# meyerls/FruitNeRF

Measured on AMD Instinct MI355X. Metric: train rays/sec, fruit_nerf on synthetic apple 800x800, higher is better.
Workload: dtype f32 fwd (MLP GEMMs: 3-piece bf16 split, 6 products, ~2^-24) / 2-piece bwd (dX, dW: 3 products, ~2^-17; its forward recompute 3-piece); everything else f32

## Files before the change

fruitnerf_amd/csrc/hash_scatter.hip:

```cpp
#include <stdlib.h>
#include <string.h>

#include "hash_scatter.hpp"
#include "sequencer.hpp"

namespace fnr {

constexpr int SC_MAX_ROWS = 8192;
constexpr int SC_MAX_BINS = 256;
constexpr int SC_CHUNK = 512;
constexpr int SC_EMIT_THREADS = 512;
constexpr int SC_PER_THREAD = SC_CHUNK / SC_EMIT_THREADS;
constexpr int SC_BINS_PER_THREAD = 1;
static_assert(SC_MAX_BINS <= SC_EMIT_THREADS, "one bin per thread");
constexpr int SC_CNT_STRIDE = 32;

__device__ unsigned long long g_scatter_overflow_records;
__device__ unsigned long long g_scatter_records[2][64][16];



struct ScatterPlan {
  int log2_rows;
  int bins_per_level;
// ... 52 lines not shown
  bool any_run;
};
template <int CTRL>
__device__ __forceinline__ float dpp_shr0_f32(float v) {
  return __builtin_bit_cast(float, __builtin_amdgcn_update_dpp(0, __builtin_bit_cast(int, v), CTRL, 0xf, 0xf, true));
}
__device__ __forceinline__ RunMasks run_structure(uint32_t key_a, uint32_t key_b, int lane) {
  const int j = lane & 15;
  const uint32_t pa = dpp_u32<0x111>(~key_a, key_a), pb = dpp_u32<0x111>(key_b, key_b);
  const bool head = (pa != key_a) || (pb != key_b);
  const unsigned long long heads = __ballot(head);
  const uint32_t row = (uint32_t)(heads >> (lane & 48)) & 0xffffu;
  const uint32_t below = row & ((2u << j) - 1u);
  const int dist = j - (31 - __clz((int)below));
  RunMasks m;
  m.g1 = dist >= 1 ? 1.0f : 0.0f;
  m.g2 = dist >= 2 ? 1.0f : 0.0f;
  m.g4 = dist >= 4 ? 1.0f : 0.0f;
  m.g8 = dist >= 8 ? 1.0f : 0.0f;
  m.tail = (j == 15) || ((row >> (j + 1)) & 1u);
  m.any_run = ~heads != 0ull;
  return m;
}
__device__ __forceinline__ float run_sum(float v, const RunMasks& m) {
  v = fmaf(m.g1, dpp_shr0_f32<0x111>(v), v);
  v = fmaf(m.g2, dpp_shr0_f32<0x112>(v), v);
  v = fmaf(m.g4, dpp_shr0_f32<0x114>(v), v);
  v = fmaf(m.g8, dpp_shr0_f32<0x118>(v), v);
  return v;
}



template <class Source, bool PAIRS>
__global__ __launch_bounds__(SC_EMIT_THREADS) void k_scatter_emit(GridDev grid, Warp warp, Source src, long long N,
                                                      const float2* __restrict__ d_feats, float2* __restrict__ queue_v,
                                                      unsigned short* __restrict__ queue_r, unsigned* __restrict__ qcount, unsigned* __restrict__ qmax,
                                                      long long cap, int log2_rows, int level0, int level_count, int lpb
                                                      ) {
  __shared__ float2 s_val[SC_CHUNK * 8];
  __shared__ unsigned s_key[SC_CHUNK * 8];
  __shared__ unsigned s_cnt[SC_MAX_BINS];
  __shared__ unsigned s_off[SC_MAX_BINS];
  __shared__ unsigned s_base[SC_MAX_BINS];
  __shared__ unsigned s_max;
  __shared__ unsigned s_wsum[SC_EMIT_THREADS / 64];
  const int bins = 1 << (grid.log2_T - log2_rows);
  const int lane = threadIdx.x & 63, wave = threadIdx.x >> 6;
  const uint32_t mask = (1u << grid.log2_T) - 1u;
  const uint32_t row_mask = (1u << log2_rows) - 1u;
  const long long n0 = (long long)blockIdx.x * SC_CHUNK;
  static_assert(SC_PER_THREAD == 1, "one sample per thread");
  const long long n = n0 + threadIdx.x;
  const bool valid = n < N;
  float x[3] = {0.f, 0.f, 0.f};
  float2 gf_next = make_float2(0.f, 0.f);
  const int lrel0 = blockIdx.y * lpb;
  if (valid) {
    gf_next = ntc_load<NT_DFEATS_LD>(&d_feats[(size_t)(level0 + lrel0) * N + n]);
    float px, py, pz;
    src.position(n, px, py, pz);
    warp_position(warp, px, py, pz, x);
  }
  for (int li = 0; li < lpb && lrel0 + li < level_count; ++li) {
  const int lrel = lrel0 + li;
  const int level = level0 + lrel;
  for (int i = threadIdx.x; i < bins; i += SC_EMIT_THREADS) {
    s_cnt[i] = 0;
  }
  if (threadIdx.x == 0) s_max = 0;
  __syncthreads();
  const int scaling = grid.scalings[level];
  const float2 gf = gf_next;
  if (valid && li + 1 < lpb && lrel + 1 < level_count) gf_next = ntc_load<NT_DFEATS_LD>(&d_feats[(size_t)(level + 1) * N + n]);

  uint32_t hk[SC_PER_THREAD][8];
  float vxk[SC_PER_THREAD][8], vyk[SC_PER_THREAD][8];
  float tmax = 0.0f;
  unsigned emit_mask[SC_PER_THREAD];
#pragma unroll
  for (int q = 0; q < SC_PER_THREAD; ++q) {
    float wgt[8];
    const GridLevel g = corner_weights(x, scaling, mask, hk[q], wgt);
    const uint32_t key_a = valid ? (g.f[0] | (g.f[1] << 16)) : 0xffffffffu;
    const uint32_t key_b = valid ? (g.f[2] | ((g.c[0] - g.f[0]) << 16) | ((g.c[1] - g.f[1]) << 17) |
                                    ((g.c[2] - g.f[2]) << 18))
                                 : (0x80000000u | (uint32_t)lane);
    const RunMasks rm = run_structure(key_a, key_b, lane);
    emit_mask[q] = 0;
#pragma unroll
    for (int k = 0; k < 8; ++k) {
      vxk[q][k] = valid ? wgt[k] * gf.x : 0.0f;
      vyk[q][k] = valid ? wgt[k] * gf.y : 0.0f;
    }
    if (rm.any_run) {
// ... 84 lines not shown
#pragma unroll
      for (int k = 0; k < 8; ++k) {
        if ((emit_mask[q] >> k) & 1u) {
          const int bin = hk[q][k] >> log2_rows;
          const unsigned pos = s_off[bin] + atomicAdd(&s_cnt[bin], 1u);
          s_val[pos] = make_float2(vxk[q][k], vyk[q][k]);
          s_key[pos] = (hk[q][k] & row_mask) | ((unsigned)bin << 16);
        }
      }
    }
  }
  __syncthreads();
  float* table = reinterpret_cast<float*>(grid.table + ((size_t)level << grid.log2_T));
  unsigned overflowed_here = 0;
  for (unsigned i = threadIdx.x; i < total; i += SC_EMIT_THREADS) {
    const float2 v = s_val[i];
    const unsigned key = s_key[i];
    const unsigned bin = key >> 16, row_in_bin = key & 0xffffu;
    const unsigned slot = s_base[bin] + (i - s_off[bin]);
    if ((long long)slot < cap) {
      const size_t q = ((size_t)lrel * bins + bin) * cap + slot;
      queue_v[q] = v;
      queue_r[q] = (unsigned short)row_in_bin;
    } else {
      qmax[(size_t)lrel * SC_CNT_STRIDE + 1] = 1u;
      ++overflowed_here;
      const size_t row = ((size_t)bin << log2_rows) + row_in_bin;
      atomicAdd(table + 2 * row, v.x);
      atomicAdd(table + 2 * row + 1, v.y);
    }
  }
  if (overflowed_here) atomicAdd(&g_scatter_overflow_records, (unsigned long long)overflowed_here);
  __syncthreads();
  }
}

__device__ __forceinline__ void acc_record(unsigned long long* __restrict__ s_acc, unsigned row, const float2& v,
                                           double scale) {
  const long long ix = __double2ll_rn((double)v.x * scale), iy = __double2ll_rn((double)v.y * scale);
  atomicAdd(&s_acc[2 * row], (unsigned long long)ix);
  atomicAdd(&s_acc[2 * row + 1], (unsigned long long)iy);
}

template <bool ADAM>
__device__ __forceinline__ void accumulate_bin(const AccArgs& A, int vblock, unsigned long long* __restrict__ s_acc) {
  const GridDev& grid = A.grid;
  const float2* __restrict__ queue_v = A.queue_v;
  const unsigned short* __restrict__ queue_r = A.queue_r;
  unsigned* __restrict__ qcount = A.qcount;
  unsigned* __restrict__ qmax = A.qmax;
  unsigned* __restrict__ qdone = A.qdone;
  const long long cap = A.cap;
  const int log2_rows = A.log2_rows, level0 = A.level0;
  const TableAdam& adam = A.adam;
  const int rows = 1 << log2_rows;
  const int bins = 1 << (grid.log2_T - log2_rows);
  const int gbin = A.nbins - 1 - vblock;
  const int lrel = gbin / bins, bin = gbin - lrel * bins;
  const int level = level0 + lrel;
  long long n = qcount[(size_t)gbin * SC_CNT_STRIDE];
  const float vmax = __uint_as_float(qmax[(size_t)lrel * SC_CNT_STRIDE]);
  const bool overflowed = qmax[(size_t)lrel * SC_CNT_STRIDE + 1] != 0u;
  {
    const unsigned held_n = (unsigned)n, held_max = __float_as_uint(vmax), held_ovf = overflowed ? 1u : 0u;
    asm volatile("s_waitcnt vmcnt(0) lgkmcnt(0)" ::"v"(held_n), "v"(held_max), "v"(held_ovf) : "memory");
  }
// ... 103 lines not shown
      }
      float2 P = adam.p[row0 + e2], M = adam.m[row0 + e2], V = adam.v[row0 + e2];
      table_adam_update(adam, g.x, P.x, M.x, V.x);
      table_adam_update(adam, g.y, P.y, M.y, V.y);
      adam.p[row0 + e2] = P;
      adam.m[row0 + e2] = M;
      adam.v[row0 + e2] = V;
    }
  } else {
    for (int e2 = threadIdx.x; e2 < rows; e2 += blockDim.x) {
      const long long ax = (long long)s_acc[2 * e2], ay = (long long)s_acc[2 * e2 + 1];
      if (ax != 0 || ay != 0) {
        float2 t = dst[e2];
        t.x += (float)((double)ax * inv);
        t.y += (float)((double)ay * inv);
        dst[e2] = t;
      }
    }
  }
}

extern __shared__ __attribute__((aligned(16))) unsigned char acc_smem[];
template <bool ADAM>
__global__ __launch_bounds__(1024) void k_scatter_accumulate(AccArgs a) {
  accumulate_bin<ADAM>(a, (int)blockIdx.x, reinterpret_cast<unsigned long long*>(acc_smem));
}
template <bool ADAM>
__global__ __launch_bounds__(1024) void k_scatter_accumulate2(AccArgs a, AccArgs b) {
  unsigned long long* s_acc = reinterpret_cast<unsigned long long*>(acc_smem);
  if ((int)blockIdx.x < a.nbins) accumulate_bin<ADAM>(a, (int)blockIdx.x, s_acc);
  else accumulate_bin<ADAM>(b, (int)blockIdx.x - a.nbins, s_acc);
}

int scatter_emit(const fnr_grid* grid_grad, const Warp& warp, const RaySource& src, long long N, const float2* d_feats,
                 int level0, int level_count, void* workspace, size_t workspace_bytes, int workspace_clean, hipStream_t st,
                 const TableAdam* adam, AccArgs& acc) {
  FNR_CHECK_ARG(level0 >= 0 && level_count >= 1 && level0 + level_count <= grid_grad->n_levels,
                "hash scatter: level range [%d,+%d) outside the %d levels", level0, level_count, grid_grad->n_levels);
  const ScatterPlan p = scatter_plan(N, level_count, grid_grad->log2_hashmap_size);
  FNR_CHECK_ARG(p.bins_per_level <= SC_MAX_BINS, "hash scatter: log2_hashmap_size %d too large for the bin histogram",
                grid_grad->log2_hashmap_size);
  FNR_CHECK_ARG(workspace && workspace_bytes >= p.count_bytes + p.queue_bytes, "hash scatter: workspace too small");
  unsigned* qcount = reinterpret_cast<unsigned*>(workspace);
  float2* queue_v = reinterpret_cast<float2*>(reinterpret_cast<char*>(workspace) + p.count_bytes);
  unsigned short* queue_r = reinterpret_cast<unsigned short*>(reinterpret_cast<char*>(workspace) + p.count_bytes + p.value_bytes);
  if (!workspace_clean) FNR_HIP(hipMemsetAsync(qcount, 0, p.count_bytes, st));
  const size_t nbins_all = (size_t)level_count * p.bins_per_level;
  const long long chunks = (N + SC_CHUNK - 1) / SC_CHUNK;
  FNR_CHECK_ARG(chunks < (1ll << 31), "hash scatter: too many samples");
  const GridDev gd = make_grid(grid_grad);
  for (int l = 0; l < grid_grad->n_levels; ++l)
    FNR_CHECK_ARG(gd.scalings[l] > 0 && gd.scalings[l] < 65535, "hash scatter: level resolution %d out of range", gd.scalings[l]);
  bool pairs = true;
  for (int l = level0; l < level0 + level_count; ++l) pairs = pairs && gd.scalings[l] < (1 << p.log2_rows);
  int lpb = 1;
  {
    const char* e = getenv("FNR_EMIT_LPB");
    const int forced = e ? atoi(e) : 0;
    const long long slots = 3ll * device_cu_count();
    while (lpb < level_count && lpb < 8 && chunks * ((level_count + 2 * lpb - 1) / (2 * lpb)) >= 2 * slots) lpb *= 2;
    if (forced > 0) lpb = forced;
    if (lpb > level_count) lpb = level_count;
  }
  const unsigned gy = (unsigned)((level_count + lpb - 1) / lpb);
  if (chunks != 0)
    hipLaunchKernelGGL((pairs ? k_scatter_emit<RaySource, true> : k_scatter_emit<RaySource, false>), dim3((unsigned)chunks, gy),
                       dim3(SC_EMIT_THREADS), 0, st, gd, warp, src, N, d_feats, queue_v, queue_r, qcount,
                       qcount + nbins_all * SC_CNT_STRIDE, p.cap, p.log2_rows, level0, level_count, lpb);
  FNR_LAUNCH_CHECK();
  acc.grid = gd;
  acc.queue_v = queue_v, acc.queue_r = queue_r, acc.qcount = qcount;
  acc.qmax = qcount + nbins_all * SC_CNT_STRIDE;
  acc.qdone = qcount + (nbins_all + level_count) * SC_CNT_STRIDE;
  acc.cap = p.cap, acc.log2_rows = p.log2_rows, acc.level0 = level0;
  acc.nbins = level_count * p.bins_per_level;
  acc.kind = 0;
  acc.adam = adam ? *adam : TableAdam{};
  return FNR_OK;
}

static int acc_lds_bytes(const AccArgs& a) { return (2 << a.log2_rows) * (int)sizeof(unsigned long long); }
constexpr int ACC_MAX_LDS = 2 * SC_MAX_ROWS * (int)sizeof(unsigned long long);

int scatter_accumulate(const AccArgs& a, bool adam, hipStream_t st) {
  const int rc = adam ? ensure_dyn_lds<k_scatter_accumulate<true>>(ACC_MAX_LDS) : ensure_dyn_lds<k_scatter_accumulate<false>>(ACC_MAX_LDS);
  if (rc) return rc;
  hipLaunchKernelGGL((adam ? k_scatter_accumulate<true> : k_scatter_accumulate<false>), dim3((unsigned)a.nbins), dim3(1024),
                     acc_lds_bytes(a), st, a);
  FNR_LAUNCH_CHECK();
  return FNR_OK;
}

int scatter_accumulate2(const AccArgs& a, const AccArgs& b, bool adam, hipStream_t st) {
  const int bytes = acc_lds_bytes(a) > acc_lds_bytes(b) ? acc_lds_bytes(a) : acc_lds_bytes(b);
  const int rc = adam ? ensure_dyn_lds<k_scatter_accumulate2<true>>(ACC_MAX_LDS) : ensure_dyn_lds<k_scatter_accumulate2<false>>(ACC_MAX_LDS);
  if (rc) return rc;
  hipLaunchKernelGGL((adam ? k_scatter_accumulate2<true> : k_scatter_accumulate2<false>), dim3((unsigned)(a.nbins + b.nbins)),
                     dim3(1024), bytes, st, a, b);
  FNR_LAUNCH_CHECK();
  return FNR_OK;
}

static int binned_scatter(const fnr_grid* grid_grad, const Warp& warp, const RaySource& src, long long N,
                          const float2* d_feats, int level0, int level_count, void* workspace, size_t workspace_bytes,
                          int workspace_clean, hipStream_t st, const TableAdam* adam = nullptr) {
  AccArgs acc;
  const int rc = scatter_emit(grid_grad, warp, src, N, d_feats, level0, level_count, workspace, workspace_bytes,
                              workspace_clean, st, adam, acc);
  if (rc) return rc;
  return scatter_accumulate(acc, adam != nullptr, st);
}

}

using namespace fnr;


extern "C" int fnr_debug_scatter_overflows(uint64_t* count_host, int reset) {
  FNR_CHECK_ARG(count_host, "debug_scatter_overflows: null argument");
  unsigned long long n = 0;
  FNR_HIP(hipMemcpyFromSymbol(&n, HIP_SYMBOL(g_scatter_overflow_records), sizeof(n)));
  *count_host = n;
  if (reset) {
    n = 0;
    FNR_HIP(hipMemcpyToSymbol(HIP_SYMBOL(g_scatter_overflow_records), &n, sizeof(n)));
  }
// ... 67 lines not shown
```

fruitnerf_amd/csrc/hash_scatter.hpp:

```cpp
#pragma once
#include "hash_sources.hpp"

namespace fnr {

struct AccArgs {
  GridDev grid;
  const float2* queue_v;
  const unsigned short* queue_r;
  unsigned *qcount, *qmax, *qdone;
  long long cap;
  int log2_rows, level0, nbins;
  int kind;
  TableAdam adam;
};

#pragma GCC visibility push(hidden)
int scatter_emit(const fnr_grid* grid_grad, const Warp& warp, const RaySource& src, long long N, const float2* d_feats,
                 int level0, int level_count, void* workspace, size_t workspace_bytes, int workspace_clean, hipStream_t st,
                 const TableAdam* adam, AccArgs& acc);
int scatter_accumulate(const AccArgs& a, bool adam, hipStream_t st);
int scatter_accumulate2(const AccArgs& a, const AccArgs& b, bool adam, hipStream_t st);
#pragma GCC visibility pop

}
```

fruitnerf_amd/csrc/prop_bwd.hip:

```cpp
#include <stdlib.h>

#include "hash_scatter.hpp"
#include "sequencer.hpp"

namespace fnr {

constexpr int PROP_PART = 320;

template <int L, int H, bool POSGRAD>
__global__ __launch_bounds__(256) void k_prop_bwd(GridDev grid, float4* __restrict__ d_xw, Warp warp, RaySource src,
                                                  long long N, const float* __restrict__ w0,
                                                  const float* __restrict__ b0, const float* __restrict__ w1,
                                                  const float* __restrict__ b1, const float2* __restrict__ feat_save,
                                                  const float* __restrict__ d_density, float2* __restrict__ d_feats,
                                                  float* __restrict__ partials) {
  constexpr int K = 2 * L;
  __shared__ float s_dh[256][H + 1];
  __shared__ float s_ha[256][H + 1];
  __shared__ float s_f[256][K + 1];
  __shared__ float s_do[256];
  static_assert(H == 16 && K <= 16, "phase 2 is a single 16x16 MFMA tile");
  using f32x4 = __attribute__((ext_vector_type(4))) float;
  const int tid = threadIdx.x;
  const int lane = tid & 63, wave = tid >> 6;
  const int j = lane & 15, g = lane >> 4;
  f32x4 d1 = {0.f, 0.f, 0.f, 0.f}, d2 = {0.f, 0.f, 0.f, 0.f}, d3 = {0.f, 0.f, 0.f, 0.f};
  float db1 = 0.0f;
  const float ones_col0 = (j == 0) ? 1.0f : 0.0f;
  const long long n_iter = (N + 255) / 256;
  for (long long it = blockIdx.x; it < n_iter; it += gridDim.x) {
    const long long n = it * 256 + tid;
    float f[K], dout = 0.0f;
#pragma unroll
    for (int k = 0; k < K; ++k) f[k] = 0.0f;
    bool sel = false;
    float x[3] = {0.f, 0.f, 0.f};
    if (n < N) {
      float px, py, pz;
      src.position(n, px, py, pz);
      sel = warp_position(warp, px, py, pz, x);
// ... 69 lines not shown
      const float bf = (j < K) ? s_f[row][j < K ? j : 0] : 0.0f;
      d1 = __builtin_amdgcn_mfma_f32_16x16x4f32(a1, bf, d1, 0, 0, 0);
      d2 = __builtin_amdgcn_mfma_f32_16x16x4f32(a2, ones_col0, d2, 0, 0, 0);
      d3 = __builtin_amdgcn_mfma_f32_16x16x4f32(a1, ones_col0, d3, 0, 0, 0);
    }
    __syncthreads();
  }
  float* red = &s_dh[0][0];
#pragma unroll
  for (int r = 0; r < 4; ++r) {
    red[((wave * 3 + 0) * 16 + 4 * g + r) * 16 + j] = d1[r];
    red[((wave * 3 + 1) * 16 + 4 * g + r) * 16 + j] = d2[r];
    red[((wave * 3 + 2) * 16 + 4 * g + r) * 16 + j] = d3[r];
  }
  db1 = wave_sum(db1);
  if (lane == 0) s_do[wave] = db1;
  __syncthreads();
  {
    const int o = tid >> 4, k = tid & 15;
    auto total = [&](int which) {
      return (red[((0 * 3 + which) * 16 + o) * 16 + k] + red[((1 * 3 + which) * 16 + o) * 16 + k]) +
             (red[((2 * 3 + which) * 16 + o) * 16 + k] + red[((3 * 3 + which) * 16 + o) * 16 + k]);
    };
    float* part = partials + (size_t)blockIdx.x * PROP_PART;
    part[tid] = total(0);
    if (k == 0) {
      part[256 + o] = total(1);
      part[272 + o] = total(2);
    }
    if (tid == 0) part[288] = (s_do[0] + s_do[1]) + (s_do[2] + s_do[3]);
  }
}

constexpr int PRD_E = 16, PRD_Y = 64;
struct PropReduceArgs {
  const float* partials;
  int nblocks, K;
  float *g_w0, *g_b0, *g_w1, *g_b1;
  WeightAdam wa;
};
template <bool ADAM>
__device__ __forceinline__ void prop_reduce_block(int block, const PropReduceArgs& a) {
  __shared__ float s_part[PRD_Y][PRD_E];
  const float* __restrict__ partials = a.partials;
  const int nblocks = a.nblocks, K = a.K;
  const int t = threadIdx.x % PRD_E, y = threadIdx.x / PRD_E;
  const int e = block * PRD_E + t;
  float s = 0.0f;
  if (e <= 288) {
    int b = y;
    for (; b + 7 * PRD_Y < nblocks; b += 8 * PRD_Y) {
      float v[8];
#pragma unroll
      for (int u = 0; u < 8; ++u) v[u] = partials[(size_t)(b + u * PRD_Y) * PROP_PART + e];
#pragma unroll
      for (int u = 0; u < 8; ++u) s += v[u];
    }
    for (; b < nblocks; b += PRD_Y) s += partials[(size_t)b * PROP_PART + e];
  }
  s_part[y][t] = s;
  __syncthreads();
  if (y != 0 || e > 288) return;
#pragma unroll 8
  for (int q = 1; q < PRD_Y; ++q) s += s_part[q][t];
  if (!ADAM && s == 0.0f) return;
  float* dst = nullptr;
  if (e < 256) {
    const int o = e >> 4, k = e & 15;
    if (k < K) dst = &a.g_w0[o * K + k];
  } else if (e < 272) {
    dst = &a.g_w1[e - 256];
  } else if (e < 288) {
    dst = &a.g_b0[e - 272];
  } else {
    dst = &a.g_b1[0];
  }
  if (!dst) return;
  if constexpr (ADAM) weight_adam_entry(a.wa, dst, s);
  else *dst += s;
}
template <bool ADAM>
__global__ __launch_bounds__(PRD_E * PRD_Y) void k_prop_reduce(PropReduceArgs a) {
  prop_reduce_block<ADAM>((int)blockIdx.x, a);
}
template <bool ADAM>
__global__ __launch_bounds__(PRD_E * PRD_Y) void k_prop_reduce2(PropReduceArgs a, PropReduceArgs b) {
  constexpr int NB = PROP_PART / PRD_E;
  if ((int)blockIdx.x < NB) prop_reduce_block<ADAM>((int)blockIdx.x, a);
  else prop_reduce_block<ADAM>((int)blockIdx.x - NB, b);
}

struct PropLevel {
  const fnr_prop_net *net, *grads;
  const fnr_warp* warp;
  const float* euclid;
  int S;
  const float *feat_save, *d_density;
  float* d_position;
  void* workspace;
  size_t workspace_bytes;
  int workspace_clean;
  const fnr_table_adam* table_adam;
  long long N;
  TableAdam ta{};
  WeightAdam wa{};
};

static size_t prop_dfeat_bytes(int L, long long N) { return ((size_t)L * (size_t)N * sizeof(float2) + 255) / 256 * 256; }
static size_t prop_partial_bytes() { return (size_t)3 * device_cu_count() * PROP_PART * sizeof(float); }

static int prop_level_check(const char* who, PropLevel& lv, const fnr_rays* rays, const fnr_table_adam* weight_adam,
                            const float* grad_arena) {
  FNR_CHECK_ARG(lv.net && lv.grads && lv.warp && rays && lv.euclid && lv.feat_save && lv.d_density && lv.workspace && lv.S > 0,
                "%s: null argument", who);
  if (lv.table_adam) {
    FNR_CHECK_ARG(weight_adam && grad_arena, "%s: weight_adam / grad_arena missing", who);
    int rc = make_table_adam(weight_adam, lv.wa.t);
    if (rc) return rc;
    lv.wa.p_off = weight_adam->params - grad_arena;
    lv.wa.m_off = weight_adam->exp_avg - grad_arena;
    lv.wa.v_off = weight_adam->exp_avg_sq - grad_arena;
    rc = make_table_adam(lv.table_adam, lv.ta);
// ... 10 lines not shown
                "%s: workspace too small", who);
  return FNR_OK;
}

static int prop_mlp_bwd(const PropLevel& lv, const fnr_rays* rays, hipStream_t st, PropReduceArgs& red) {
  const int L = lv.net->grid.n_levels;
  static const int cap_per_cu = [] { const char* e = getenv("FNR_PROP_BWD_WGS_PER_CU"); const int v = e ? atoi(e) : 0; return (v >= 1 && v <= 3) ? v : 3; }();
  const long long capped = (long long)cap_per_cu * device_cu_count();
  const long long blocks = (lv.N + 255) / 256 < capped ? (lv.N + 255) / 256 : capped;
  float2* d_feats = reinterpret_cast<float2*>(lv.workspace);
  float* partials = reinterpret_cast<float*>(reinterpret_cast<char*>(lv.workspace) + prop_dfeat_bytes(L, lv.N));
  float4* d_xw = reinterpret_cast<float4*>(lv.d_position);
  decltype(&k_prop_bwd<1, 16, true>) kernel = nullptr;
  switch (L) {
#define FNR_PROPB_CASE(LL) case LL: kernel = d_xw ? k_prop_bwd<LL, 16, true> : k_prop_bwd<LL, 16, false>; break;
    FNR_PROPB_CASE(1) FNR_PROPB_CASE(2) FNR_PROPB_CASE(3) FNR_PROPB_CASE(4)
    FNR_PROPB_CASE(5) FNR_PROPB_CASE(6) FNR_PROPB_CASE(7) FNR_PROPB_CASE(8)
#undef FNR_PROPB_CASE
  }
  hipLaunchKernelGGL(kernel, dim3((unsigned)blocks), dim3(256), 0, st, make_grid(&lv.net->grid), d_xw, make_warp(lv.warp),
                     RaySource{make_rays(rays), lv.euclid, lv.S}, lv.N, lv.net->w0, lv.net->b0, lv.net->w1, lv.net->b1,
                     reinterpret_cast<const float2*>(lv.feat_save), lv.d_density, d_feats, partials);
  FNR_LAUNCH_CHECK();
  red = PropReduceArgs{partials, (int)blocks, 2 * L, lv.grads->w0, lv.grads->b0, lv.grads->w1, lv.grads->b1, lv.wa};
  return FNR_OK;
}

static int prop_reduce(const PropReduceArgs& red, bool adam, hipStream_t st) {
  hipLaunchKernelGGL((adam ? k_prop_reduce<true> : k_prop_reduce<false>), dim3(PROP_PART / PRD_E), dim3(PRD_E * PRD_Y), 0, st, red);
  FNR_LAUNCH_CHECK();
  return FNR_OK;
}

static int prop_emit(const PropLevel& lv, const fnr_rays* rays, hipStream_t st, AccArgs& acc) {
  const int L = lv.net->grid.n_levels;
  const size_t used = prop_dfeat_bytes(L, lv.N) + prop_partial_bytes();
  const int rc = scatter_emit(&lv.grads->grid, make_warp(lv.warp), RaySource{make_rays(rays), lv.euclid, lv.S}, lv.N,
                              reinterpret_cast<const float2*>(lv.workspace), 0, L, reinterpret_cast<char*>(lv.workspace) + used,
                              lv.workspace_bytes - used, lv.workspace_clean, st, lv.table_adam ? &lv.ta : nullptr, acc);
  acc.kind = 1;
  return rc;
}

static int prop_single(const char* who, PropLevel lv, const fnr_rays* rays, const fnr_table_adam* weight_adam,
                       const float* grad_arena, void* stream) {
  int rc = prop_level_check(who, lv, rays, weight_adam, grad_arena);
  if (rc || lv.N == 0) return rc;
  FNR_PROF(OP_PROP_BWD, lv.N);
  const hipStream_t st = as_stream(stream);
  const bool adam = lv.table_adam != nullptr;
  PropReduceArgs red;
  AccArgs acc;
  if ((rc = prop_mlp_bwd(lv, rays, st, red)) || (rc = prop_reduce(red, adam, st)) || (rc = prop_emit(lv, rays, st, acc))) return rc;
  return scatter_accumulate(acc, adam, st);
}

template <class Again>
static int pair_begin(const char* name, Again again, void* event, PropLevel (&lv)[2], const fnr_prop_net* const* nets,
                      const fnr_prop_net* const* grads, const fnr_warp* const* warps, const fnr_rays* rays,
                      const float* const* euclid_bins, const int* S, const float* const* feat_save,
                      const float* const* d_density, float* const* d_position, const fnr_table_adam* const* table_adam,
                      const fnr_table_adam* weight_adam, const float* grad_arena, void* const* workspace,
                      const size_t* workspace_bytes, const int* workspace_clean, void* stream) {
  if (seq::recording() && nets && grads && warps && rays && euclid_bins && S && feat_save && d_density && d_position &&
      workspace && workspace_bytes && workspace_clean && nets[0] && nets[1] && grads[0] && grads[1] && warps[0] && warps[1]) {
    struct Pair {
      fnr_prop_net net[2], grad[2];
      fnr_warp warp[2];
      fnr_rays rays;
      const float *euclid[2], *feat[2], *dd[2];
      float* dpos[2];
      fnr_table_adam tadam[2], wadam;
// ... 7 lines not shown
      p.feat[q] = feat_save[q], p.dd[q] = d_density[q], p.dpos[q] = d_position[q], p.ws[q] = workspace[q];
      p.ws_bytes[q] = workspace_bytes[q], p.ws_clean[q] = workspace_clean[q];
    }
    p.rays = *rays;
    p.has_adam = table_adam && table_adam[0] && table_adam[1] && weight_adam;
    if (p.has_adam) p.tadam[0] = *table_adam[0], p.tadam[1] = *table_adam[1], p.wadam = *weight_adam;
    seq::push(name, [=](const fnr_step_scalars* sc) {
      const fnr_prop_net* n_[2] = {&p.net[0], &p.net[1]};
      const fnr_prop_net* g_[2] = {&p.grad[0], &p.grad[1]};
      const fnr_warp* w_[2] = {&p.warp[0], &p.warp[1]};
      const fnr_table_adam t0 = seq::patched(p.tadam[0], sc), t1 = seq::patched(p.tadam[1], sc), wa = seq::patched(p.wadam, sc);
      const fnr_table_adam* t_[2] = {&t0, &t1};
      return again(event, n_, g_, w_, &p.rays, p.euclid, p.S, p.feat, p.dd, p.dpos, p.has_adam ? t_ : nullptr,
                   p.has_adam ? &wa : nullptr, grad_arena, p.ws, p.ws_bytes, p.ws_clean, stream);
    });
  }
  const char* who = name + 4;
  FNR_CHECK_ARG(nets && grads && warps && rays && euclid_bins && S && feat_save && d_density && d_position && workspace &&
                    workspace_bytes && workspace_clean,
                "%s: null argument", who);
  FNR_CHECK_ARG(nets[0] != nets[1] && grads[0] != grads[1] && workspace[0] != workspace[1],
                "%s: the two levels must have their own network, gradients and workspace", who);
  const bool adam = table_adam && table_adam[0] && table_adam[1];
  FNR_CHECK_ARG(adam || !(table_adam && (table_adam[0] || table_adam[1])), "%s: one table_adam missing", who);
  for (int q = 0; q < 2 && rays->n_rays != 0; ++q) {
    lv[q] = PropLevel{nets[q], grads[q], warps[q], euclid_bins[q], S[q], feat_save[q], d_density[q], d_position[q], workspace[q],
                      workspace_bytes[q], workspace_clean[q], adam ? table_adam[q] : nullptr};
    const int rc = prop_level_check(who, lv[q], rays, weight_adam, grad_arena);
    if (rc) return rc;
  }
  return FNR_OK;
}

static int pair_accumulate(const PropLevel (&lv)[2], const AccArgs (&acc)[2], hipStream_t st) {
  const bool first_longer = lv[0].S >= lv[1].S;
  return scatter_accumulate2(first_longer ? acc[0] : acc[1], first_longer ? acc[1] : acc[0], lv[0].table_adam != nullptr, st);
}

}

using namespace fnr;

extern "C" size_t fnr_prop_density_bwd_workspace_bytes(int64_t n_samples, int n_levels, int log2_hashmap_size) {
  return prop_dfeat_bytes(n_levels, n_samples) + prop_partial_bytes() +
         fnr_hash_scatter_workspace_bytes(n_samples, n_levels, log2_hashmap_size);
}

extern "C" int fnr_prop_density_bwd(const fnr_prop_net* net, const fnr_prop_net* grads, const fnr_warp* warp,
                                    const fnr_rays* rays, const float* euclid_bins, int S, const float* feat_save,
                                    const float* d_density, float* d_position, void* workspace,
                                    size_t workspace_bytes, int workspace_clean, void* stream) {
  FNR_SEQ_UNRECORDABLE("fnr_prop_density_bwd");
  return prop_single("prop_density_bwd", PropLevel{net, grads, warp, euclid_bins, S, feat_save, d_density, d_position, workspace,
                                                   workspace_bytes, workspace_clean, nullptr},
                     rays, nullptr, nullptr, stream);
}

extern "C" int fnr_prop_density_bwd_adam(const fnr_prop_net* net, const fnr_prop_net* grads, const fnr_warp* warp,
                                         const fnr_rays* rays, const float* euclid_bins, int S, const float* feat_save,
                                         const float* d_density, float* d_position, const fnr_table_adam* table_adam,
                                         const fnr_table_adam* weight_adam, const float* grad_arena, void* workspace,
                                         size_t workspace_bytes, int workspace_clean, void* stream) {
  FNR_SEQ_UNRECORDABLE("fnr_prop_density_bwd_adam");
  FNR_CHECK_ARG(table_adam && weight_adam && grad_arena, "prop_density_bwd_adam: optimiser descriptors missing");
  return prop_single("prop_density_bwd_adam", PropLevel{net, grads, warp, euclid_bins, S, feat_save, d_density, d_position,
                                                        workspace, workspace_bytes, workspace_clean, table_adam},
                     rays, weight_adam, grad_arena, stream);
}

extern "C" int fnr_prop_density_bwd_pair(const fnr_prop_net* const* nets, const fnr_prop_net* const* grads,
                                         const fnr_warp* const* warps, const fnr_rays* rays,
                                         const float* const* euclid_bins, const int* S, const float* const* feat_save,
                                         const float* const* d_density, float* const* d_position,
                                         const fnr_table_adam* const* table_adam, const fnr_table_adam* weight_adam,
                                         const float* grad_arena, void* const* workspace, const size_t* workspace_bytes,
                                         const int* workspace_clean, void* stream) {
  PropLevel lv[2];
  int rc = pair_begin("fnr_prop_density_bwd_pair", [](void*, auto... args) { return fnr_prop_density_bwd_pair(args...); }, nullptr,
                      lv, nets, grads, warps, rays, euclid_bins, S, feat_save, d_density, d_position, table_adam, weight_adam,
                      grad_arena, workspace, workspace_bytes, workspace_clean, stream);
  if (rc || rays->n_rays == 0) return rc;
  FNR_PROF(OP_PROP_BWD, rays->n_rays * ((long long)S[0] + (long long)S[1]));
  const hipStream_t st = as_stream(stream);
  AccArgs acc[2];
  for (int q = 0; q < 2; ++q) {
    PropReduceArgs red;
    if ((rc = prop_mlp_bwd(lv[q], rays, st, red)) || (rc = prop_reduce(red, lv[q].table_adam != nullptr, st)) ||
        (rc = prop_emit(lv[q], rays, st, acc[q])))
      return rc;
  }
  return pair_accumulate(lv, acc, st);
}

extern "C" int fnr_prop_density_bwd_pair_split(const fnr_prop_net* const* nets, const fnr_prop_net* const* grads,
                                               const fnr_warp* const* warps, const fnr_rays* rays,
                                               const float* const* euclid_bins, const int* S, const float* const* feat_save,
                                               const float* const* d_density, float* const* d_position,
                                               const fnr_table_adam* const* table_adam, const fnr_table_adam* weight_adam,
                                               const float* grad_arena, void* const* workspace, const size_t* workspace_bytes,
                                               const int* workspace_clean, void* stream, void* position_ready_event) {
  PropLevel lv[2];
  int rc = pair_begin("fnr_prop_density_bwd_pair_split",
                      [](void* ev, auto... args) { return fnr_prop_density_bwd_pair_split(args..., ev); }, position_ready_event,
                      lv, nets, grads, warps, rays, euclid_bins, S, feat_save, d_density, d_position, table_adam, weight_adam,
                      grad_arena, workspace, workspace_bytes, workspace_clean, stream);
  if (rc) return rc;
  const hipStream_t st = as_stream(stream);
  const hipEvent_t position_ready = reinterpret_cast<hipEvent_t>(position_ready_event);
  if (rays->n_rays == 0) {
    if (position_ready) FNR_HIP(hipEventRecord(position_ready, st));
    return FNR_OK;
  }
  FNR_PROF(OP_PROP_BWD, rays->n_rays * ((long long)S[0] + (long long)S[1]));
  PropReduceArgs red[2];
  for (int q = 0; q < 2; ++q)
    if ((rc = prop_mlp_bwd(lv[q], rays, st, red[q]))) return rc;
  if (position_ready) FNR_HIP(hipEventRecord(position_ready, st));
  hipLaunchKernelGGL((lv[0].table_adam ? k_prop_reduce2<true> : k_prop_reduce2<false>), dim3(2 * (PROP_PART / PRD_E)),
                     dim3(PRD_E * PRD_Y), 0, st, red[0], red[1]);
  FNR_LAUNCH_CHECK();
  AccArgs acc[2];
  for (int q = 0; q < 2; ++q)
    if ((rc = prop_emit(lv[q], rays, st, acc[q]))) return rc;
  return pair_accumulate(lv, acc, st);
}
```

Baseline: 6.165 million.

## Fuse proposal weight reduction and both levels' hash emits into one launch

Merges the two proposal networks' scatter-emit kernels and the MLP weight-gradient reduction into one kernel with a flattened grid. Workgroups are dispatched by index to emit level A, emit level B, or a reduction slice that reuses the emit LDS staging. The levels-per-workgroup heuristic is now computed over both emits jointly. The intent is to cut launch overhead and fill the device better with small independent kernels running side by side. The trade-off is that the reduction now runs at 512-thread granularity inside a kernel sized for the emit's LDS. It also adds a debug env hook that dumps bin counts.

```diff
diff --git a/fruitnerf_amd/csrc/hash_scatter.hip b/fruitnerf_amd/csrc/hash_scatter.hip
--- a/fruitnerf_amd/csrc/hash_scatter.hip
+++ b/fruitnerf_amd/csrc/hash_scatter.hip
@@ -108,35 +108,50 @@
 
 
 
+struct EmitLds {
+  float2* val;
+  unsigned *key, *cnt, *off, *base, *max, *wsum;
+};
+#define FNR_EMIT_LDS                                                                                                   \
+  __shared__ float2 s_val[SC_CHUNK * 8];                                                   \
+  __shared__ unsigned s_key[SC_CHUNK * 8];                                         \
+  __shared__ unsigned s_cnt[SC_MAX_BINS];                                      \
+  __shared__ unsigned s_off[SC_MAX_BINS];                                      \
+  __shared__ unsigned s_base[SC_MAX_BINS];                                  \
+  __shared__ unsigned s_max;                 \
+  __shared__ unsigned s_wsum[SC_EMIT_THREADS / 64];                                                                    \
+  const EmitLds lds { s_val, s_key, s_cnt, s_off, s_base, &s_max, s_wsum }
+
 template <class Source, bool PAIRS>
-__global__ __launch_bounds__(SC_EMIT_THREADS) void k_scatter_emit(GridDev grid, Warp warp, Source src, long long N,
-                                                      const float2* __restrict__ d_feats, float2* __restrict__ queue_v,
-                                                      unsigned short* __restrict__ queue_r, unsigned* __restrict__ qcount, unsigned* __restrict__ qmax,
-                                                      long long cap, int log2_rows, int level0, int level_count, int lpb
-                                                      ) {
-  __shared__ float2 s_val[SC_CHUNK * 8];
-  __shared__ unsigned s_key[SC_CHUNK * 8];
-  __shared__ unsigned s_cnt[SC_MAX_BINS];
-  __shared__ unsigned s_off[SC_MAX_BINS];
-  __shared__ unsigned s_base[SC_MAX_BINS];
-  __shared__ unsigned s_max;
-  __shared__ unsigned s_wsum[SC_EMIT_THREADS / 64];
+__device__ __forceinline__ void emit_chunk(const EmitArgs<Source>& E, unsigned chunk, unsigned ly, const EmitLds& lds) {
+  const GridDev& grid = E.grid;
+  const Source& src = E.src;
+  const long long N = E.N, cap = E.cap;
+  const float2* __restrict__ d_feats = E.d_feats;
+  float2* __restrict__ queue_v = E.queue_v;
+  unsigned short* __restrict__ queue_r = E.queue_r;
+  unsigned* __restrict__ qcount = E.qcount;
+  unsigned* __restrict__ qmax = E.qmax;
+  const int log2_rows = E.log2_rows, level0 = E.level0, level_count = E.level_count, lpb = E.lpb;
+  float2* s_val = lds.val;
+  unsigned *s_key = lds.key, *s_cnt = lds.cnt, *s_off = lds.off, *s_base = lds.base, *s_wsum = lds.wsum;
+  unsigned& s_max = *lds.max;
   const int bins = 1 << (grid.log2_T - log2_rows);
   const int lane = threadIdx.x & 63, wave = threadIdx.x >> 6;
   const uint32_t mask = (1u << grid.log2_T) - 1u;
   const uint32_t row_mask = (1u << log2_rows) - 1u;
-  const long long n0 = (long long)blockIdx.x * SC_CHUNK;
+  const long long n0 = (long long)chunk * SC_CHUNK;
   static_assert(SC_PER_THREAD == 1, "one sample per thread");
   const long long n = n0 + threadIdx.x;
   const bool valid = n < N;
   float x[3] = {0.f, 0.f, 0.f};
   float2 gf_next = make_float2(0.f, 0.f);
-  const int lrel0 = blockIdx.y * lpb;
+  const int lrel0 = (int)ly * lpb;
   if (valid) {
     gf_next = ntc_load<NT_DFEATS_LD>(&d_feats[(size_t)(level0 + lrel0) * N + n]);
     float px, py, pz;
     src.position(n, px, py, pz);
-    warp_position(warp, px, py, pz, x);
+    warp_position(E.warp, px, py, pz, x);
   }
   for (int li = 0; li < lpb && lrel0 + li < level_count; ++li) {
   const int lrel = lrel0 + li;
@@ -287,6 +302,33 @@
   }
   if (overflowed_here) atomicAdd(&g_scatter_overflow_records, (unsigned long long)overflowed_here);
   __syncthreads();
+  }
+}
+
+template <class Source, bool PAIRS>
+__global__ __launch_bounds__(SC_EMIT_THREADS) void k_scatter_emit(EmitArgs<Source> e) {
+  FNR_EMIT_LDS;
+  emit_chunk<Source, PAIRS>(e, blockIdx.x, blockIdx.y, lds);
+}
+constexpr int EMIT2_RED_E = SC_EMIT_THREADS / PRD_Y;
+static_assert(sizeof(float) * PRD_Y * EMIT2_RED_E <= sizeof(float2) * SC_CHUNK * 8, "the reduction's slices fit the record staging");
+template <bool PAIRS>
+__global__ __launch_bounds__(SC_EMIT_THREADS) void k_prop_bwd_pair_emit(EmitArgs<RaySource> a, EmitArgs<RaySource> b, PropReduceArgs ra,
+                                                                  PropReduceArgs rb, int adam) {
+  FNR_EMIT_LDS;
+  constexpr unsigned NB = PROP_PART / EMIT2_RED_E;
+  const unsigned na = a.chunks * a.gy, nb = b.chunks * b.gy;
+  unsigned i = blockIdx.x;
+  if (i < na) {
+    emit_chunk<RaySource, PAIRS>(a, i % a.chunks, i / a.chunks, lds);
+  } else if ((i -= na) < nb) {
+    emit_chunk<RaySource, PAIRS>(b, i % b.chunks, i / b.chunks, lds);
+  } else {
+    i -= nb;
+    float(*s_part)[EMIT2_RED_E] = reinterpret_cast<float(*)[EMIT2_RED_E]>(s_val);
+    const PropReduceArgs& r = i < NB ? ra : rb;
+    if (adam) prop_reduce_block<true, EMIT2_RED_E>((int)(i < NB ? i : i - NB), r, s_part);
+    else prop_reduce_block<false, EMIT2_RED_E>((int)(i < NB ? i : i - NB), r, s_part);
   }
 }
 
@@ -456,9 +498,9 @@
   else accumulate_bin<ADAM>(b, (int)blockIdx.x - a.nbins, s_acc);
 }
 
-int scatter_emit(const fnr_grid* grid_grad, const Warp& warp, const RaySource& src, long long N, const float2* d_feats,
-                 int level0, int level_count, void* workspace, size_t workspace_bytes, int workspace_clean, hipStream_t st,
-                 const TableAdam* adam, AccArgs& acc) {
+int scatter_emit_plan(const fnr_grid* grid_grad, const Warp& warp, const RaySource& src, long long N, const float2* d_feats,
+                      int level0, int level_count, void* workspace, size_t workspace_bytes, int workspace_clean, hipStream_t st,
+                      const TableAdam* adam, EmitArgs<RaySource>& em, AccArgs& acc) {
   FNR_CHECK_ARG(level0 >= 0 && level_count >= 1 && level0 + level_count <= grid_grad->n_levels,
                 "hash scatter: level range [%d,+%d) outside the %d levels", level0, level_count, grid_grad->n_levels);
   const ScatterPlan p = scatter_plan(N, level_count, grid_grad->log2_hashmap_size);
@@ -477,21 +519,8 @@
     FNR_CHECK_ARG(gd.scalings[l] > 0 && gd.scalings[l] < 65535, "hash scatter: level resolution %d out of range", gd.scalings[l]);
   bool pairs = true;
   for (int l = level0; l < level0 + level_count; ++l) pairs = pairs && gd.scalings[l] < (1 << p.log2_rows);
-  int lpb = 1;
-  {
-    const char* e = getenv("FNR_EMIT_LPB");
-    const int forced = e ? atoi(e) : 0;
-    const long long slots = 3ll * device_cu_count();
-    while (lpb < level_count && lpb < 8 && chunks * ((level_count + 2 * lpb - 1) / (2 * lpb)) >= 2 * slots) lpb *= 2;
-    if (forced > 0) lpb = forced;
-    if (lpb > level_count) lpb = level_count;
-  }
-  const unsigned gy = (unsigned)((level_count + lpb - 1) / lpb);
-  if (chunks != 0)
-    hipLaunchKernelGGL((pairs ? k_scatter_emit<RaySource, true> : k_scatter_emit<RaySource, false>), dim3((unsigned)chunks, gy),
-                       dim3(SC_EMIT_THREADS), 0, st, gd, warp, src, N, d_feats, queue_v, queue_r, qcount,
-                       qcount + nbins_all * SC_CNT_STRIDE, p.cap, p.log2_rows, level0, level_count, lpb);
-  FNR_LAUNCH_CHECK();
+  em = EmitArgs<RaySource>{gd, warp, src, N, p.cap, d_feats, queue_v, queue_r, qcount, qcount + nbins_all * SC_CNT_STRIDE,
+                           p.log2_rows, level0, level_count, 1, (unsigned)chunks, (unsigned)level_count, pairs};
   acc.grid = gd;
   acc.queue_v = queue_v, acc.queue_r = queue_r, acc.qcount = qcount;
   acc.qmax = qcount + nbins_all * SC_CNT_STRIDE;
@@ -503,6 +532,53 @@
   return FNR_OK;
 }
 
+static void emit_levels_per_workgroup(EmitArgs<RaySource>* const* em, int n) {
+  const char* e = getenv("FNR_EMIT_LPB");
+  const int forced = e ? atoi(e) : 0;
+  const long long slots = 3ll * device_cu_count();
+  int lpb = 1, most_levels = 0;
+  for (int q = 0; q < n; ++q) most_levels = em[q]->level_count > most_levels ? em[q]->level_count : most_levels;
+  auto workgroups = [&](int per) {
+    long long w = 0;
+    for (int q = 0; q < n; ++q) w += (long long)em[q]->chunks * ((em[q]->level_count + per - 1) / per);
+    return w;
+  };
+  while (lpb < most_levels && lpb < 8 && workgroups(2 * lpb) >= 2 * slots) lpb *= 2;
+  if (forced > 0) lpb = forced;
+  for (int q = 0; q < n; ++q) {
+    em[q]->lpb = lpb > em[q]->level_count ? em[q]->level_count : lpb;
+    em[q]->gy = (unsigned)((em[q]->level_count + em[q]->lpb - 1) / em[q]->lpb);
+  }
+}
+
+int scatter_emit(const fnr_grid* grid_grad, const Warp& warp, const RaySource& src, long long N, const float2* d_feats,
+                 int level0, int level_count, void* workspace, size_t workspace_bytes, int workspace_clean, hipStream_t st,
+                 const TableAdam* adam, AccArgs& acc) {
+  EmitArgs<RaySource> em;
+  const int rc = scatter_emit_plan(grid_grad, warp, src, N, d_feats, level0, level_count, workspace, workspace_bytes,
+                                   workspace_clean, st, adam, em, acc);
+  if (rc) return rc;
+  EmitArgs<RaySource>* const one[1] = {&em};
+  emit_levels_per_workgroup(one, 1);
+  if (em.chunks != 0)
+    hipLaunchKernelGGL((em.pairs ? k_scatter_emit<RaySource, true> : k_scatter_emit<RaySource, false>), dim3(em.chunks, em.gy),
+                       dim3(SC_EMIT_THREADS), 0, st, em);
+  FNR_LAUNCH_CHECK();
+  return FNR_OK;
+}
+
+int scatter_emit2(EmitArgs<RaySource>& a, EmitArgs<RaySource>& b, const PropReduceArgs& ra, const PropReduceArgs& rb, bool adam,
+                  hipStream_t st) {
+  EmitArgs<RaySource>* const both[2] = {&a, &b};
+  emit_levels_per_workgroup(both, 2);
+  const long long workgroups = (long long)a.chunks * a.gy + (long long)b.chunks * b.gy + 2 * (PROP_PART / EMIT2_RED_E);
+  FNR_CHECK_ARG(workgroups < (1ll << 31), "hash scatter: too many samples");
+  hipLaunchKernelGGL((a.pairs && b.pairs ? k_prop_bwd_pair_emit<true> : k_prop_bwd_pair_emit<false>), dim3((unsigned)workgroups),
+                     dim3(SC_EMIT_THREADS), 0, st, a, b, ra, rb, adam ? 1 : 0);
+  FNR_LAUNCH_CHECK();
+  return FNR_OK;
+}
+
 static int acc_lds_bytes(const AccArgs& a) { return (2 << a.log2_rows) * (int)sizeof(unsigned long long); }
 constexpr int ACC_MAX_LDS = 2 * SC_MAX_ROWS * (int)sizeof(unsigned long long);
 
@@ -515,7 +591,29 @@
   return FNR_OK;
 }
 
+static int dump_bin_counts(const AccArgs& a, hipStream_t st, const char* path) {
+  const size_t words = (size_t)a.nbins * SC_CNT_STRIDE;
+  unsigned* host = static_cast<unsigned*>(malloc(words * sizeof(unsigned)));
+  FNR_CHECK_ARG(host, "hash scatter: no memory for the bin counts");
+  const hipError_t e1 = hipMemcpyAsync(host, a.qcount, words * sizeof(unsigned), hipMemcpyDeviceToHost, st);
+  const hipError_t e2 = e1 == hipSuccess ? hipStreamSynchronize(st) : e1;
+  FILE* f = e2 == hipSuccess ? fopen(path, "a") : nullptr;
+  if (f) {
+    fprintf(f, "%d %d %d %lld", a.kind, 1 << (a.grid.log2_T - a.log2_rows), a.nbins, a.cap);
+    for (int i = 0; i < a.nbins; ++i) fprintf(f, " %u", host[(size_t)i * SC_CNT_STRIDE]);
+    fprintf(f, "\n");
+    fclose(f);
+  }
+  free(host);
+  FNR_HIP(e2);
+  return FNR_OK;
+}
+
 int scatter_accumulate2(const AccArgs& a, const AccArgs& b, bool adam, hipStream_t st) {
+  if (const char* path = getenv("FNR_SCATTER_DUMP_COUNTS")) {
+    int rc;
+    if ((rc = dump_bin_counts(a, st, path)) || (rc = dump_bin_counts(b, st, path))) return rc;
+  }
   const int bytes = acc_lds_bytes(a) > acc_lds_bytes(b) ? acc_lds_bytes(a) : acc_lds_bytes(b);
   const int rc = adam ? ensure_dyn_lds<k_scatter_accumulate2<true>>(ACC_MAX_LDS) : ensure_dyn_lds<k_scatter_accumulate2<false>>(ACC_MAX_LDS);
   if (rc) return rc;
diff --git a/fruitnerf_amd/csrc/hash_scatter.hpp b/fruitnerf_amd/csrc/hash_scatter.hpp
--- a/fruitnerf_amd/csrc/hash_scatter.hpp
+++ b/fruitnerf_amd/csrc/hash_scatter.hpp
@@ -1,5 +1,6 @@
 #pragma once
 #include "hash_sources.hpp"
+#include "prop_reduce.hpp"
 
 namespace fnr {
 
@@ -14,10 +15,31 @@
   TableAdam adam;
 };
 
+template <class Source>
+struct EmitArgs {
+  GridDev grid;
+  Warp warp;
+  Source src;
+  long long N, cap;
+  const float2* d_feats;
+  float2* queue_v;
+  unsigned short* queue_r;
+  unsigned *qcount, *qmax;
+  int log2_rows, level0, level_count;
+  int lpb;
+  unsigned chunks, gy;
+  bool pairs;
+};
+
 #pragma GCC visibility push(hidden)
 int scatter_emit(const fnr_grid* grid_grad, const Warp& warp, const RaySource& src, long long N, const float2* d_feats,
                  int level0, int level_count, void* workspace, size_t workspace_bytes, int workspace_clean, hipStream_t st,
                  const TableAdam* adam, AccArgs& acc);
+int scatter_emit_plan(const fnr_grid* grid_grad, const Warp& warp, const RaySource& src, long long N, const float2* d_feats,
+                      int level0, int level_count, void* workspace, size_t workspace_bytes, int workspace_clean, hipStream_t st,
+                      const TableAdam* adam, EmitArgs<RaySource>& em, AccArgs& acc);
+int scatter_emit2(EmitArgs<RaySource>& a, EmitArgs<RaySource>& b, const PropReduceArgs& ra, const PropReduceArgs& rb, bool adam,
+                  hipStream_t st);
 int scatter_accumulate(const AccArgs& a, bool adam, hipStream_t st);
 int scatter_accumulate2(const AccArgs& a, const AccArgs& b, bool adam, hipStream_t st);
 #pragma GCC visibility pop
diff --git a/fruitnerf_amd/csrc/prop_bwd.hip b/fruitnerf_amd/csrc/prop_bwd.hip
--- a/fruitnerf_amd/csrc/prop_bwd.hip
+++ b/fruitnerf_amd/csrc/prop_bwd.hip
@@ -1,11 +1,10 @@
 #include <stdlib.h>
 
 #include "hash_scatter.hpp"
+#include "prop_reduce.hpp"
 #include "sequencer.hpp"
 
 namespace fnr {
-
-constexpr int PROP_PART = 320;
 
 template <int L, int H, bool POSGRAD>
 __global__ __launch_bounds__(256) void k_prop_bwd(GridDev grid, float4* __restrict__ d_xw, Warp warp, RaySource src,
@@ -141,62 +140,11 @@
   }
 }
 
-constexpr int PRD_E = 16, PRD_Y = 64;
-struct PropReduceArgs {
-  const float* partials;
-  int nblocks, K;
-  float *g_w0, *g_b0, *g_w1, *g_b1;
-  WeightAdam wa;
-};
-template <bool ADAM>
-__device__ __forceinline__ void prop_reduce_block(int block, const PropReduceArgs& a) {
-  __shared__ float s_part[PRD_Y][PRD_E];
-  const float* __restrict__ partials = a.partials;
-  const int nblocks = a.nblocks, K = a.K;
-  const int t = threadIdx.x % PRD_E, y = threadIdx.x / PRD_E;
-  const int e = block * PRD_E + t;
-  float s = 0.0f;
-  if (e <= 288) {
-    int b = y;
-    for (; b + 7 * PRD_Y < nblocks; b += 8 * PRD_Y) {
-      float v[8];
-#pragma unroll
-      for (int u = 0; u < 8; ++u) v[u] = partials[(size_t)(b + u * PRD_Y) * PROP_PART + e];
-#pragma unroll
-      for (int u = 0; u < 8; ++u) s += v[u];
-    }
-    for (; b < nblocks; b += PRD_Y) s += partials[(size_t)b * PROP_PART + e];
-  }
-  s_part[y][t] = s;
-  __syncthreads();
-  if (y != 0 || e > 288) return;
-#pragma unroll 8
-  for (int q = 1; q < PRD_Y; ++q) s += s_part[q][t];
-  if (!ADAM && s == 0.0f) return;
-  float* dst = nullptr;
-  if (e < 256) {
-    const int o = e >> 4, k = e & 15;
-    if (k < K) dst = &a.g_w0[o * K + k];
-  } else if (e < 272) {
-    dst = &a.g_w1[e - 256];
-  } else if (e < 288) {
-    dst = &a.g_b0[e - 272];
-  } else {
-    dst = &a.g_b1[0];
-  }
-  if (!dst) return;
-  if constexpr (ADAM) weight_adam_entry(a.wa, dst, s);
-  else *dst += s;
-}
+constexpr int PRD_E = 16;
 template <bool ADAM>
 __global__ __launch_bounds__(PRD_E * PRD_Y) void k_prop_reduce(PropReduceArgs a) {
-  prop_reduce_block<ADAM>((int)blockIdx.x, a);
-}
-template <bool ADAM>
-__global__ __launch_bounds__(PRD_E * PRD_Y) void k_prop_reduce2(PropReduceArgs a, PropReduceArgs b) {
-  constexpr int NB = PROP_PART / PRD_E;
-  if ((int)blockIdx.x < NB) prop_reduce_block<ADAM>((int)blockIdx.x, a);
-  else prop_reduce_block<ADAM>((int)blockIdx.x - NB, b);
+  __shared__ float s_part[PRD_Y][PRD_E];
+  prop_reduce_block<ADAM, PRD_E>((int)blockIdx.x, a, s_part);
 }
 
 struct PropLevel {
@@ -273,12 +221,17 @@
   return FNR_OK;
 }
 
-static int prop_emit(const PropLevel& lv, const fnr_rays* rays, hipStream_t st, AccArgs& acc) {
+static int prop_emit(const PropLevel& lv, const fnr_rays* rays, hipStream_t st, AccArgs& acc, EmitArgs<RaySource>* em = nullptr) {
   const int L = lv.net->grid.n_levels;
   const size_t used = prop_dfeat_bytes(L, lv.N) + prop_partial_bytes();
-  const int rc = scatter_emit(&lv.grads->grid, make_warp(lv.warp), RaySource{make_rays(rays), lv.euclid, lv.S}, lv.N,
-                              reinterpret_cast<const float2*>(lv.workspace), 0, L, reinterpret_cast<char*>(lv.workspace) + used,
-                              lv.workspace_bytes - used, lv.workspace_clean, st, lv.table_adam ? &lv.ta : nullptr, acc);
+  const RaySource src{make_rays(rays), lv.euclid, lv.S};
+  const float2* d_feats = reinterpret_cast<const float2*>(lv.workspace);
+  void* ws = reinterpret_cast<char*>(lv.workspace) + used;
+  const TableAdam* ta = lv.table_adam ? &lv.ta : nullptr;
+  const int rc = em ? scatter_emit_plan(&lv.grads->grid, make_warp(lv.warp), src, lv.N, d_feats, 0, L, ws, lv.workspace_bytes - used,
+                                        lv.workspace_clean, st, ta, *em, acc)
+                    : scatter_emit(&lv.grads->grid, make_warp(lv.warp), src, lv.N, d_feats, 0, L, ws, lv.workspace_bytes - used,
+                                   lv.workspace_clean, st, ta, acc);
   acc.kind = 1;
   return rc;
 }
@@ -352,9 +305,16 @@
   return FNR_OK;
 }
 
-static int pair_accumulate(const PropLevel (&lv)[2], const AccArgs (&acc)[2], hipStream_t st) {
-  const bool first_longer = lv[0].S >= lv[1].S;
-  return scatter_accumulate2(first_longer ? acc[0] : acc[1], first_longer ? acc[1] : acc[0], lv[0].table_adam != nullptr, st);
+static int pair_scatter(const PropLevel (&lv)[2], const PropReduceArgs (&red)[2], const fnr_rays* rays, hipStream_t st) {
+  AccArgs acc[2];
+  EmitArgs<RaySource> em[2];
+  int rc;
+  for (int q = 0; q < 2; ++q)
+    if ((rc = prop_emit(lv[q], rays, st, acc[q], &em[q]))) return rc;
+  const int f = lv[0].S >= lv[1].S ? 0 : 1;
+  const bool adam = lv[0].table_adam != nullptr;
+  if ((rc = scatter_emit2(em[f], em[1 - f], red[f], red[1 - f], adam, st))) return rc;
+  return scatter_accumulate2(acc[f], acc[1 - f], adam, st);
 }
 
 }
@@ -402,14 +362,10 @@
   if (rc || rays->n_rays == 0) return rc;
   FNR_PROF(OP_PROP_BWD, rays->n_rays * ((long long)S[0] + (long long)S[1]));
   const hipStream_t st = as_stream(stream);
-  AccArgs acc[2];
-  for (int q = 0; q < 2; ++q) {
-    PropReduceArgs red;
-    if ((rc = prop_mlp_bwd(lv[q], rays, st, red)) || (rc = prop_reduce(red, lv[q].table_adam != nullptr, st)) ||
-        (rc = prop_emit(lv[q], rays, st, acc[q])))
-      return rc;
-  }
-  return pair_accumulate(lv, acc, st);
+  PropReduceArgs red[2];
+  for (int q = 0; q < 2; ++q)
+    if ((rc = prop_mlp_bwd(lv[q], rays, st, red[q]))) return rc;
+  return pair_scatter(lv, red, rays, st);
 }
 
 extern "C" int fnr_prop_density_bwd_pair_split(const fnr_prop_net* const* nets, const fnr_prop_net* const* grads,
@@ -436,11 +392,5 @@
   for (int q = 0; q < 2; ++q)
     if ((rc = prop_mlp_bwd(lv[q], rays, st, red[q]))) return rc;
   if (position_ready) FNR_HIP(hipEventRecord(position_ready, st));
-  hipLaunchKernelGGL((lv[0].table_adam ? k_prop_reduce2<true> : k_prop_reduce2<false>), dim3(2 * (PROP_PART / PRD_E)),
-                     dim3(PRD_E * PRD_Y), 0, st, red[0], red[1]);
-  FNR_LAUNCH_CHECK();
-  AccArgs acc[2];
-  for (int q = 0; q < 2; ++q)
-    if ((rc = prop_emit(lv[q], rays, st, acc[q]))) return rc;
-  return pair_accumulate(lv, acc, st);
-}
+  return pair_scatter(lv, red, rays, st);
+}
diff --git a/fruitnerf_amd/csrc/prop_reduce.hpp b/fruitnerf_amd/csrc/prop_reduce.hpp
--- /dev/null
+++ b/fruitnerf_amd/csrc/prop_reduce.hpp
@@ -0,0 +1,56 @@
+#pragma once
+#include "common.hpp"
+
+namespace fnr {
+
+constexpr int PROP_PART = 320;
+
+constexpr int PRD_Y = 64;
+struct PropReduceArgs {
+  const float* partials;
+  int nblocks, K;
+  float *g_w0, *g_b0, *g_w1, *g_b1;
+  WeightAdam wa;
+};
+template <bool ADAM, int E>
+__device__ __forceinline__ void prop_reduce_block(int block, const PropReduceArgs& a, float (*s_part)[E]) {
+  static_assert(PROP_PART % E == 0, "whole workgroups");
+  const float* __restrict__ partials = a.partials;
+  const int nblocks = a.nblocks, K = a.K;
+  const int t = threadIdx.x % E, y = threadIdx.x / E;
+  const int e = block * E + t;
+  float s = 0.0f;
+  if (e <= 288) {
+    int b = y;
+    for (; b + 7 * PRD_Y < nblocks; b += 8 * PRD_Y) {
+      float v[8];
+#pragma unroll
+      for (int u = 0; u < 8; ++u) v[u] = partials[(size_t)(b + u * PRD_Y) * PROP_PART + e];
+#pragma unroll
+      for (int u = 0; u < 8; ++u) s += v[u];
+    }
+    for (; b < nblocks; b += PRD_Y) s += partials[(size_t)b * PROP_PART + e];
+  }
+  s_part[y][t] = s;
+  __syncthreads();
+  if (y != 0 || e > 288) return;
+#pragma unroll 8
+  for (int q = 1; q < PRD_Y; ++q) s += s_part[q][t];
+  if (!ADAM && s == 0.0f) return;
+  float* dst = nullptr;
+  if (e < 256) {
+    const int o = e >> 4, k = e & 15;
+    if (k < K) dst = &a.g_w0[o * K + k];
+  } else if (e < 272) {
+    dst = &a.g_w1[e - 256];
+  } else if (e < 288) {
+    dst = &a.g_b0[e - 272];
+  } else {
+    dst = &a.g_b1[0];
+  }
+  if (!dst) return;
+  if constexpr (ADAM) weight_adam_entry(a.wa, dst, s);
+  else *dst += s;
+}
+
+}
```

Result: faster. 6.234 million (median of 6 runs) (+1.1%).
